# aanna0701/face-recognition-pytorch

Hardware: AMD Instinct MI355X
Metric: train imgs/sec IR-50-layout ResNet50 + ArcFace/PartialFC head, 112x112 (higher is better)
Workload: dtype bf16

## Files before the change

### face-recognition-pytorch_amd/frhip/csrc/igemm_halo.h

```cpp
#pragma once
#include <type_traits>
#include "igemm_nt.h"

#ifndef FRHIP_ABL
#define FRHIP_ABL 0
#endif

namespace frhip {

struct HaloGeom {
    int H, W, C;
    int M, Nout, Ktot;
    int sign;
    uint32_t a_bytes, b_bytes;
    const float* xf_scale;
    const float* xf_shift;
    void* xf_out;
    FastDiv d_hw, d_w;
};

template <typename T, int WM, int WN, int MT, int HBUFS>
struct HaloTile {
    static constexpr int WAVES = WM * WN, THREADS = 64 * WAVES;
    static constexpr int WROWS = MT * 16, BM = WM * WROWS, BN = WN * 64;
    static constexpr int BKE = NT_ROWB / (int)sizeof(T);
    static constexpr int MAXW = 56;
    static constexpr int HROWS = ((BM + 2 * MAXW + 2 + 7) / 8) * 8;
    static constexpr int ZROW = HROWS * NT_ROWB;
    static constexpr int HALO_BYTES = ZROW + NT_ROWB;
    static constexpr int WBUF_BYTES = BN * NT_ROWB;
    static constexpr int DUMP_OFF = HBUFS * HALO_BYTES;
    static constexpr int W_OFF = DUMP_OFF + 1024;
    static constexpr int WRING = 3;
    static constexpr int B_PIECES = (BN / 8 + WAVES - 1) / WAVES;
    static constexpr int ITER_PIECES = B_PIECES + (HBUFS == 2 ? 1 : 0);
    template <typename TS> static constexpr int stage_pitch() { return 64 * (int)sizeof(TS) + 16; }
    template <typename TS> static constexpr int lds_bytes() {
        constexpr int loop = W_OFF + WRING * WBUF_BYTES;
        constexpr int epi = WAVES * WROWS * stage_pitch<TS>();
        return loop > epi ? loop : epi;
    }
};

template <typename T, int WM, int WN, int MT, int HBUFS, bool XF = false>
struct HaloMainloop {
    static_assert(!XF || (HBUFS == 1 && std::is_same<T, bf16_t>::value), "operand transform: single-buffer bf16 tile only");
    typedef HaloTile<T, WM, WN, MT, HBUFS> Tile;
    typedef typename Mma<T>::Frag Frag;
    static constexpr int BM = Tile::BM, BN = Tile::BN, BKE = Tile::BKE;

    f32x4_t acc[4][MT];

    __device__ __forceinline__ void run(const HaloGeom& g, const void* __restrict__ a_ptr,
                                        const void* __restrict__ b_ptr, char* smem, int mtile, int ntile) {
        const int lane = lane_id(), wave = wave_id();
        const int wm = wave / WN, wn = wave % WN;
        const __amdgpu_buffer_rsrc_t ra = make_rsrc(a_ptr, g.a_bytes);
        const __amdgpu_buffer_rsrc_t rb = make_rsrc(b_ptr, g.b_bytes);
        const int m0 = mtile * BM;
        const int hrows = BM + 2 * g.W + 2;
        const int npieces = (hrows + 7) >> 3;
        const int p_lo = m0 - g.W - 1;
        const int sub = lane >> 3;
        const uint32_t chunk_bytes = (uint32_t)(((lane & 7) ^ sub) * 16);
        const int nchunks = g.C / BKE;

        const uint32_t row0_off = (uint32_t)((p_lo + sub) * g.C) * (uint32_t)sizeof(T) + chunk_bytes;
        auto halo_piece = [&](int hb, int piece, int c0) {
            const uint32_t off = row0_off + (uint32_t)(piece * 8 * g.C + c0) * (uint32_t)sizeof(T);
            glds16(ra, smem + hb * Tile::HALO_BYTES + piece * 1024, off);
        };
        auto xform_chunk = [&](int c0) {
            if constexpr (XF) {
                const int lc = (lane & 7) ^ sub;
                float sc[8], sh[8];
#pragma unroll
                for (int e = 0; e < 8; ++e) { sc[e] = g.xf_scale[c0 + 8 * lc + e]; sh[e] = g.xf_shift[c0 + 8 * lc + e]; }
                const bool emit = g.xf_out != nullptr && ntile == 0;
                for (int piece = wave; piece < npieces; piece += Tile::WAVES) {
                    const int p = p_lo + piece * 8 + sub;
                    if (p >= 0 && p < g.M) {
                        bf16x8_t* a = reinterpret_cast<bf16x8_t*>(smem + piece * 1024 + lane * 16);
                        bf16x8_t v = *a;
#pragma unroll
                        for (int e = 0; e < 8; ++e) { const float o = (float)v[e] * sc[e] + sh[e]; v[e] = (bf16_t)fmaxf(o, 0.f); }
                        *a = v;
                        if (emit && p >= m0 && p < m0 + BM)
                            *reinterpret_cast<bf16x8_t*>(reinterpret_cast<bf16_t*>(g.xf_out) + (size_t)p * g.C + c0 + 8 * lc) = v;
                    }
                }
                asm volatile("s_waitcnt lgkmcnt(0)" ::: "memory");
            }
        };
        uint32_t brow_off[Tile::B_PIECES];
#pragma unroll
        for (int j = 0; j < Tile::B_PIECES; ++j) {
            const int piece = wave * Tile::B_PIECES + j;
            const int n = ntile * BN + piece * 8 + sub;
            brow_off[j] = (piece * 8 < BN && n < g.Nout) ? (uint32_t)n * (uint32_t)g.Ktot * (uint32_t)sizeof(T) + chunk_bytes
                                                         : OOB_OFFSET;
        }
        auto weights = [&](int wit) {
            const int ch = wit / 9, tap = wit - ch * 9;
            const bool live = ch < nchunks;
            const uint32_t kb = (uint32_t)(tap * g.C + ch * BKE) * (uint32_t)sizeof(T);
            char* wb = smem + Tile::W_OFF + (wit % Tile::WRING) * Tile::WBUF_BYTES;
#pragma unroll
            for (int j = 0; j < Tile::B_PIECES; ++j) {
                const int piece = wave * Tile::B_PIECES + j;
                const bool in_tile = piece * 8 < BN;
                glds16(rb, in_tile ? wb + piece * 1024 : smem + Tile::DUMP_OFF,
                       (live && in_tile && brow_off[j] != OOB_OFFSET) ? brow_off[j] + kb : OOB_OFFSET);
            }
        };

        const int fi = lane & 15, fg = lane >> 4;
        static_assert(Tile::HALO_BYTES < 65536, "packed fragment offsets");
        uint32_t xa[9][(MT + 1) / 2];
        {
            const int HW = g.H * g.W;
            uint32_t tt[9];
#pragma unroll
            for (int tap = 0; tap < 9; ++tap) {
                const int tc = g.W + 1 + g.sign * ((tap / 3 - 1) * g.W + (tap % 3 - 1));
                tt[tap] = (uint32_t)(tc * NT_ROWB) + (uint32_t)((fg ^ ((fi + tc) & 7)) << 4);
            }
            const uint32_t zoff = (uint32_t)(Tile::ZROW + (fg << 4));
#pragma unroll
            for (int mt = 0; mt < MT; ++mt) {
                const int q = wm * Tile::WROWS + mt * 16 + fi;
                const int m = m0 + q;
                int y = 0, x = 0;
                const bool live = m < g.M;
                if (live) { const int rem = m - (int)fdiv((uint32_t)m, g.d_hw) * HW; y = (int)fdiv((uint32_t)rem, g.d_w); x = rem - y * g.W; }
                const bool up = live && y > 0, dn = live && y < g.H - 1, lf = live && x > 0, rt = live && x < g.W - 1;
                const bool vy[3] = {g.sign > 0 ? up : dn, live, g.sign > 0 ? dn : up};
                const bool vx[3] = {g.sign > 0 ? lf : rt, live, g.sign > 0 ? rt : lf};
                const uint32_t aq = (uint32_t)(q * NT_ROWB);
#pragma unroll
                for (int tap = 0; tap < 9; ++tap) {
                    const bool ok = vy[tap / 3] && vx[tap % 3];
                    const uint32_t off = ok ? aq + tt[tap] : zoff;
                    if (mt & 1) xa[tap][mt >> 1] |= off << 16;
                    else xa[tap][mt >> 1] = off;
                }
            }
        }
        const int wa = (wn * 64 + fi) * NT_ROWB + ((fg ^ (fi & 7)) << 4);

        Frag xf[2][MT], wf[2][4];
        typedef const __attribute__((address_space(3))) char* lds_cp;
        typedef const __attribute__((address_space(3))) Frag* lds_fp;
        if ((uint32_t)(uintptr_t)LDS_ADDR(smem) != 0u) __builtin_trap();
        const uint32_t wa0 = (uint32_t)wa, wa1 = (uint32_t)(wa ^ 64);
        uint32_t xcur[MT];
        auto load_frags = [&](auto set_c, auto h_c, auto hb_c, auto slot_c, auto tap_c) {
            constexpr int SET = decltype(set_c)::value, HH = decltype(h_c)::value, HB = decltype(hb_c)::value,
                          SLOT = decltype(slot_c)::value, TAP = decltype(tap_c)::value;
            (void)xf; (void)wf; (void)xcur;
#pragma unroll
            for (int t = 0; t < 4; ++t) {
                if constexpr (FRHIP_ABL & 4) asm volatile("" : "=v"(wf[SET][t]));
                else wf[SET][t] = *(lds_fp)((lds_cp)(uintptr_t)(HH ? wa1 : wa0) + (Tile::W_OFF + SLOT * Tile::WBUF_BYTES + t * 16 * NT_ROWB));
            }
#pragma unroll
            for (int mt = 0; mt < MT; ++mt) {
                if constexpr (FRHIP_ABL & 4) asm volatile("" : "=v"(xf[SET][mt]));
                else {
                    if constexpr (HH == 0) {
                        if (mt & 1) asm volatile("v_lshrrev_b32 %0, 16, %1" : "=v"(xcur[mt]) : "v"(xa[TAP][mt >> 1]));
                        else asm volatile("v_and_b32 %0, 0xffff, %1" : "=v"(xcur[mt]) : "v"(xa[TAP][mt >> 1]));
                        xf[SET][mt] = *(lds_fp)((lds_cp)(uintptr_t)xcur[mt] + HB * Tile::HALO_BYTES);
                    } else {
                        xf[SET][mt] = *(lds_fp)((lds_cp)(uintptr_t)(xcur[mt] ^ 64u) + HB * Tile::HALO_BYTES);
                    }
                }
            }
        };
        auto mfma_set = [&](auto set_c) {
            constexpr int SET = decltype(set_c)::value;
#pragma unroll
            for (int mt = 0; mt < MT; ++mt)
#pragma unroll
                for (int nt = 0; nt < 4; ++nt) {
                    if constexpr (FRHIP_ABL & 2) { Frag fa = wf[SET][nt], fb = xf[SET][mt]; asm volatile("" :: "v"(fa), "v"(fb)); }
                    else Mma<T>::run(wf[SET][nt], xf[SET][mt], acc[nt][mt]);
                }
        };
        auto mfma_set_first = [&](auto set_c) {
            constexpr int SET = decltype(set_c)::value;
#pragma unroll
            for (int mt = 0; mt < MT; ++mt)
#pragma unroll
                for (int nt = 0; nt < 4; ++nt) {
                    f32x4_t z = f32x4_t{0.f, 0.f, 0.f, 0.f};
                    if constexpr (FRHIP_ABL & 2) { Frag fa = wf[SET][nt], fb = xf[SET][mt]; asm volatile("" :: "v"(fa), "v"(fb)); }
                    else Mma<T>::run(wf[SET][nt], xf[SET][mt], z);
                    acc[nt][mt] = z;
                }
        };
        auto interleave = [&]() {
            constexpr int NREAD = (4 + MT) * (int)(sizeof(Frag) / 16), NMFMA = 4 * MT * (sizeof(T) == 2 ? 1 : (sizeof(T) == 1 ? 2 : 4));
            constexpr int PER = NMFMA / NREAD > 0 ? NMFMA / NREAD : 1;
#pragma unroll
            for (int i = 0; i < NREAD; ++i) {
                __builtin_amdgcn_sched_group_barrier(0x008, PER, 0);
                __builtin_amdgcn_sched_group_barrier(0x100, 1, 0);
            }
        };
        typedef std::integral_constant<int, 0> I0;
        typedef std::integral_constant<int, 1> I1;

        if (threadIdx.x < 8 * HBUFS) {
            const int hbz = threadIdx.x >> 3;
            *reinterpret_cast<f32x4_t*>(smem + hbz * Tile::HALO_BYTES + Tile::ZROW + (threadIdx.x & 7) * 16) = f32x4_t{0.f, 0.f, 0.f, 0.f};
        }
        for (int piece = wave; piece < npieces; piece += Tile::WAVES) halo_piece(0, piece, 0);
        weights(0);
        weights(1);
        asm volatile("s_waitcnt vmcnt(0)" ::: "memory");
        xform_chunk(0);
        __syncthreads();
        load_frags(I0{}, I0{}, I0{}, I0{}, I0{});

        auto chunk_body = [&](auto hb_c, int ch) {
            constexpr int HB = decltype(hb_c)::value;
            constexpr int HBN = HBUFS == 2 ? (HB ^ 1) : 0;
            const int c0 = ch * BKE;
            const int it0 = ch * 9;
            auto tap_body = [&](auto tap_c) {
                constexpr int TAP = decltype(tap_c)::value;
                if constexpr (!(FRHIP_ABL & 8)) {
                    weights(it0 + TAP + 2);
                    if (HBUFS == 2) {
                        const int piece = TAP * Tile::WAVES + wave;
                        if (TAP < 8 && ch + 1 < nchunks && piece < npieces) halo_piece(HBN, piece, c0 + BKE);
                        else glds16(ra, smem + Tile::DUMP_OFF, OOB_OFFSET);
                    }
                }
                load_frags(I1{}, I1{}, hb_c, std::integral_constant<int, TAP % Tile::WRING>{}, tap_c);
                if (TAP == 0 && ch == 0) mfma_set_first(I0{});
                else mfma_set(I0{});
                interleave();
                if constexpr (FRHIP_ABL & 8) asm volatile("s_waitcnt vmcnt(0)" ::: "memory");
                else if constexpr (Tile::ITER_PIECES == 1) asm volatile("s_waitcnt vmcnt(1)" ::: "memory");
                else if constexpr (Tile::ITER_PIECES == 2) asm volatile("s_waitcnt vmcnt(2)" ::: "memory");
                else if constexpr (Tile::ITER_PIECES == 3) asm volatile("s_waitcnt vmcnt(3)" ::: "memory");
                else if constexpr (Tile::ITER_PIECES == 4) asm volatile("s_waitcnt vmcnt(4)" ::: "memory");
                else asm volatile("s_waitcnt vmcnt(5)" ::: "memory");
                static_assert(Tile::ITER_PIECES <= 5, "add a vmcnt case");
                if constexpr (!(FRHIP_ABL & 1)) __builtin_amdgcn_s_barrier();
                if constexpr (TAP < 8)
                    load_frags(I0{}, I0{}, hb_c, std::integral_constant<int, (TAP + 1) % Tile::WRING>{}, std::integral_constant<int, (TAP + 1) % 9>{});
                else
                    load_frags(I0{}, I0{}, std::integral_constant<int, HBN>{}, I0{}, I0{});
                mfma_set(I1{});
                interleave();
            };
            tap_body(std::integral_constant<int, 0>{}); tap_body(std::integral_constant<int, 1>{});
            tap_body(std::integral_constant<int, 2>{}); tap_body(std::integral_constant<int, 3>{});
            tap_body(std::integral_constant<int, 4>{}); tap_body(std::integral_constant<int, 5>{});
            tap_body(std::integral_constant<int, 6>{}); tap_body(std::integral_constant<int, 7>{});
            tap_body(std::integral_constant<int, 8>{});
            if (HBUFS == 1 && ch + 1 < nchunks) {
                asm volatile("s_waitcnt lgkmcnt(0)" ::: "memory");
                __builtin_amdgcn_s_barrier();
                for (int piece = wave; piece < npieces; piece += Tile::WAVES) halo_piece(0, piece, c0 + BKE);
                asm volatile("s_waitcnt vmcnt(0)" ::: "memory");
                xform_chunk(c0 + BKE);
                __builtin_amdgcn_s_barrier();
                load_frags(I0{}, I0{}, I0{}, I0{}, I0{});
            }
        };
        static_assert(HBUFS == 1 || Tile::HROWS / 8 <= 8 * Tile::WAVES, "eight halo slices must cover the halo");
        for (int ch = 0; ch < nchunks; ch += HBUFS) {
            chunk_body(std::integral_constant<int, 0>{}, ch);
            if (HBUFS == 2 && ch + 1 < nchunks) chunk_body(std::integral_constant<int, HBUFS - 1>{}, ch + 1);
        }
        asm volatile("s_waitcnt vmcnt(0)" ::: "memory");
    }

    template <typename TS>
    __device__ __forceinline__ char* stage_out(char* smem) {
        constexpr int P = Tile::template stage_pitch<TS>();
        const int lane = lane_id();
        const int fi = lane & 15, fg = lane >> 4;
        char* mine = smem + wave_id() * Tile::WROWS * P;
        __syncthreads();
#pragma unroll
        for (int nt = 0; nt < 4; ++nt)
#pragma unroll
            for (int mt = 0; mt < MT; ++mt) {
                char* p = mine + (mt * 16 + fi) * P + (nt * 16 + 4 * fg) * (int)sizeof(TS);
                if constexpr (sizeof(TS) == 4) {
                    *reinterpret_cast<f32x4_t*>(p) = acc[nt][mt];
                } else {
                    bf16x4_t v;
#pragma unroll
                    for (int e = 0; e < 4; ++e) v[e] = (bf16_t)acc[nt][mt][e];
                    *reinterpret_cast<bf16x4_t*>(p) = v;
                }
            }
        __syncthreads();
        return mine;
    }
};

}
```

### face-recognition-pytorch_amd/frhip/csrc/igemm_halo.hip

```cpp
#include "igemm_halo.h"
#include "igemm_halo_wide.h"
#include "frhip.h"

namespace frhip {

#ifndef FRHIP_CLOCK_STAMP
#define FRHIP_CLOCK_STAMP 0
#endif
#if FRHIP_CLOCK_STAMP
__device__ unsigned long long g_clock_stamps[2 * 8192];
#endif

template <typename T, int WM, int WN, int MT, int HBUFS, bool XF = false, bool LEAN = false>
__device__ __forceinline__ void halo_body(const HaloGeom& g, const void* __restrict__ a, const void* __restrict__ b,
                                          void* __restrict__ out, const void* __restrict__ res, float* __restrict__ stats,
                                          const EpiBnRed& br, char* smem, int mtile, int ntile) {
    typedef HaloTile<T, WM, WN, MT, HBUFS> Tile;
    HaloMainloop<T, WM, WN, MT, HBUFS, XF> ml;
#if FRHIP_CLOCK_STAMP
    const unsigned long long t0 = __builtin_amdgcn_s_memtime(), r0 = __builtin_amdgcn_s_memrealtime();
#endif
    ml.run(g, a, b, smem, mtile, ntile);
#if FRHIP_CLOCK_STAMP
    if (threadIdx.x == 0) {
// ... 50 lines not shown
    const int ntile = (int)(lin % (uint32_t)ntiles), mtile = (int)(lin / (uint32_t)ntiles);
    const int m_tile0 = mtile * Tile::BM;
    HaloWideMainloop ml;
#if FRHIP_CLOCK_STAMP
    const unsigned long long t0 = __builtin_amdgcn_s_memtime(), r0 = __builtin_amdgcn_s_memrealtime();
#endif
    ml.run(g, a, b, smem, m_tile0, ntile);
#if FRHIP_CLOCK_STAMP
    if (threadIdx.x == 0) {
        const unsigned long long t1 = __builtin_amdgcn_s_memtime(), r1 = __builtin_amdgcn_s_memrealtime();
        g_clock_stamps[2 * (blockIdx.x & 8191)] = t1 - t0;
        g_clock_stamps[2 * (blockIdx.x & 8191) + 1] = r1 - r0;
    }
#endif
    const int m0 = m_tile0 + wave_id() * Tile::WROWS;
#pragma unroll
    for (int half = 0; half < 2; ++half) {
        const int n0 = ntile * Tile::BN + half * 64;
        EpiOperands<T, Tile::WROWS> eo;
        if constexpr (LEAN) {
            eo.fetch_fast(res, stats ? br.y : nullptr, g.M, g.Nout, m0, n0);
            const char* mine = ml.stage_out(smem, half);
            nt_epilogue_store_fast<T, 4, 1, Tile::WROWS, Tile::THREADS, 64>(mine, Tile::stage_pitch, smem, g.M, g.Nout, out, res != nullptr,
                                                                            stats, br, eo, mtile, ntile * 2 + half);
        } else {
            eo.fetch(res, (stats || br.gelu_bwd) ? br.y : nullptr, g.M, g.Nout, m0, n0, br.res_h, br.res_w, &br.map);
            const char* mine = ml.stage_out(smem, half);
            nt_epilogue_store<T, 4, 1, Tile::WROWS, Tile::THREADS, 64>(mine, Tile::stage_pitch, smem, g.M, g.Nout, out, res != nullptr,
                                                                       stats, br, eo, mtile, ntile * 2 + half, m0, n0);
        }
    }
}

int g_epi_lean = 1;

static int halo_wide_launch(const HaloGeom& g, const void* a, const void* b, void* out, const void* res, float* stats,
                            const EpiBnRed& br, hipStream_t stream) {
    typedef HaloWideTile Tile;
    const int mtiles = (g.M + Tile::BM - 1) / Tile::BM, ntiles = (g.Nout + Tile::BN - 1) / Tile::BN;
    const bool lean = g_epi_lean && epi_lean_ok(true, g.M, g.Nout, Tile::BM, Tile::BN, br);
    auto kern = lean ? halo_wide_kernel<true> : halo_wide_kernel<false>;
    if (set_dynamic_lds(reinterpret_cast<const void*>(kern), Tile::LDS, "igemm_halo")) return FRHIP_ELAUNCH;
    hipLaunchKernelGGL(kern, dim3(mtiles * ntiles), dim3(Tile::THREADS), Tile::LDS, stream, g, a, b, out, res, stats, br, mtiles, ntiles);
    return check_launch("igemm_halo_wide");
}

template <typename T, int WM, int WN, int MT, int HBUFS, bool XF = false>
static int halo_launch(const HaloGeom& g, const void* a, const void* b, void* out, const void* res, float* stats,
                       const EpiBnRed& br, hipStream_t stream) {
    typedef HaloTile<T, WM, WN, MT, HBUFS> Tile;
    const int mtiles = (g.M + Tile::BM - 1) / Tile::BM, ntiles = (g.Nout + Tile::BN - 1) / Tile::BN;
    const int lds = Tile::template lds_bytes<T>();
    constexpr bool HAS_LEAN = sizeof(T) == 2 && WM == 4 && WN == 1 && MT == 4 && HBUFS == 1;
    bool lean = false;
    if constexpr (HAS_LEAN) lean = g_epi_lean && epi_lean_ok(true, g.M, g.Nout, Tile::BM, Tile::BN, br);
    auto kern = halo_kernel<T, WM, WN, MT, HBUFS, XF, false>;
    if constexpr (HAS_LEAN) { if (lean) kern = halo_kernel<T, WM, WN, MT, HBUFS, XF, true>; }
    if (set_dynamic_lds(reinterpret_cast<const void*>(kern), lds, "igemm_halo")) return FRHIP_ELAUNCH;
    hipLaunchKernelGGL(kern, dim3(mtiles * ntiles), dim3(Tile::THREADS), lds, stream, g, a, b, out, res, stats, br, mtiles, ntiles);
    return check_launch("igemm_halo");
}

static int g_halo_enabled = 1;

bool halo_applicable(int dtype, int h, int w, int c, int k, int r, int s, int stride, int pad) {
    const int bke = NT_ROWB / (dtype == FRHIP_DT_BF16 ? 2 : 4);
    return g_halo_enabled && r == 3 && s == 3 && stride == 1 && pad == 1 && w <= 56 && (c % bke) == 0 && (k % 8) == 0 &&
           (dtype == FRHIP_DT_BF16 || dtype == FRHIP_DT_F32);
}

static int g_halo_wide_dirs = 2;
static int halo_config(int dtype, int c, int k);
static int halo_config_w(int dtype, int w, int c, int k, int sign) {
    if ((g_halo_wide_dirs & (sign > 0 ? 1 : 2)) && dtype == FRHIP_DT_BF16 && w <= HaloWideTile::MAXW &&
        (k % 128) == 0 && (c % 64) == 0 && c >= 128 && (g_halo_enabled & 3) == 1)
        return 3;
    return halo_config(dtype, c, k);
}
static int halo_config(int dtype, int c, int k) {
    const int es = dtype == FRHIP_DT_BF16 ? 2 : 4;
    const int nchunks = c / (NT_ROWB / es);
    const bool narrow = (k % 128) != 0;
    if (dtype == FRHIP_DT_BF16) {
        const int mode = g_halo_enabled & 3;
        const bool two_per_cu = mode == 2 || (mode != 3 && nchunks <= 8);
        if (two_per_cu || narrow) return (nchunks == 1 || two_per_cu) ? 0 : 1;
        return 2;
    }
    return narrow ? 1 : 2;
}

bool halo_lean_applies(int dtype, int n, int h, int w, int c, int k, int sign) {
    if (!g_epi_lean || dtype != FRHIP_DT_BF16) return false;
    const long long M = 1LL * n * h * w;
    const int cfg = halo_config_w(dtype, w, c, k, sign) == 3 ? 3 : halo_config(dtype, c, k);
    const int bn = cfg == 3 ? HaloWideTile::BN : 64;
    if (cfg != 3 && cfg != 0) return false;
    return M % 256 == 0 && k % bn == 0 && M * k * 2 < 0x7fffffffLL;
}

int halo_stat_rows(int, int m, int, int, int, int) { return (m + 255) / 256; }

bool halo_xf_applicable(int dtype, int h, int w, int c, int k, int r, int s, int stride, int pad) {
    return dtype == FRHIP_DT_BF16 && halo_applicable(dtype, h, w, c, k, r, s, stride, pad) && halo_config(dtype, c, k) == 0;
}

int halo_run(int dtype, const void* a, const void* b, void* out, const void* res, float* stats, const EpiBnRed& br,
             int n, int h, int w, int c, int k, int sign, hipStream_t stream, const float* xf_scale, const float* xf_shift, void* xf_out) {
    const int es = dtype == FRHIP_DT_BF16 ? 2 : 4;
    const long long ab = 1LL * n * h * w * c * es, bb = 1LL * k * 9 * c * es;
    if (ab > 0x7fffffffLL || bb > 0x7fffffffLL) { set_error("igemm_halo: tensor exceeds the 2 GiB buffer window"); return FRHIP_EINVAL; }
    HaloGeom g;
    g.H = h; g.W = w; g.C = c; g.M = n * h * w; g.Nout = k; g.Ktot = 9 * c; g.sign = sign;
    g.a_bytes = (uint32_t)ab; g.b_bytes = (uint32_t)bb;
    g.xf_scale = xf_scale; g.xf_shift = xf_shift; g.xf_out = xf_out;
    g.d_hw = make_fastdiv((uint32_t)(h * w)); g.d_w = make_fastdiv((uint32_t)w);
    const int cfg = halo_config(dtype, c, k);
    if (xf_scale) {
        if (dtype != FRHIP_DT_BF16 || cfg != 0) { set_error("igemm_halo: operand transform not available for this shape"); return FRHIP_EINVAL; }
        return halo_launch<bf16_t, 4, 1, 4, 1, true>(g, a, b, out, res, stats, br, stream);
    }
    if (halo_config_w(dtype, w, c, k, sign) == 3) return halo_wide_launch(g, a, b, out, res, stats, br, stream);
    if (dtype == FRHIP_DT_BF16 && cfg == 0) return halo_launch<bf16_t, 4, 1, 4, 1>(g, a, b, out, res, stats, br, stream);
    return by_dtype(dtype, "igemm_halo", [&](auto t) {
        typedef decltype(t) T;
        return cfg == 1 ? halo_launch<T, 8, 1, 2, 2>(g, a, b, out, res, stats, br, stream)
                        : halo_launch<T, 4, 2, 4, 2>(g, a, b, out, res, stats, br, stream);
    });
}

}

#if FRHIP_CLOCK_STAMP
extern "C" int frhip_dbg_clock_read(unsigned long long* host, int pairs) {
    if (pairs > 8192) pairs = 8192;
    return hipMemcpyFromSymbol(host, HIP_SYMBOL(frhip::g_clock_stamps), sizeof(unsigned long long) * 2 * pairs) == hipSuccess ? 0 : -1;
}
#endif

extern "C" int frhip_set_epi_lean(int enabled) {
    const int old = frhip::g_epi_lean;
    if (enabled >= 0) frhip::g_epi_lean = enabled != 0;
    return old;
}

extern "C" int frhip_set_halo_wide_dirs(int dirs) {
    const int old = frhip::g_halo_wide_dirs;
    if (dirs >= 0) frhip::g_halo_wide_dirs = dirs & 3;
    return old;
}

extern "C" int frhip_set_conv_halo(int enabled) {
    const int old = frhip::g_halo_enabled;
    frhip::g_halo_enabled = enabled & 3;
    return old;
}
```

### face-recognition-pytorch_amd/frhip/csrc/igemm_nt.h

```cpp
#pragma once
#include "common.h"

namespace frhip {

struct NtGeom {
    int H, W, C;
    int Ho, Wo;
    int R, S, stride, pad;
    int mode;
    int M, Nout, Ktot;
    int ksteps, ksteps_per_split;
    uint32_t a_bytes, b_bytes;
    int par_a, par_b, hc, wc, par_r0, par_s0;
};

struct OutMap {
    int hc, wc, ho, wo, a, b;
    __device__ __forceinline__ long long row(int m) const {
        if (wc == 0) return m;
        const int per = hc * wc;
        const int img = m / per, rem = m - img * per;
        const int i = rem / wc, j = rem - i * wc;
        return ((long long)img * ho + 2 * i + a) * wo + 2 * j + b;
    }
};

constexpr int NT_ROWB = 128;

struct EpiBnRed {
    const void* y;
    const float* mean;
    const float* invstd;
    const float* mscale;
    const float* mshift;
    int res_h, res_w;
    OutMap map;
    const float* bias;
    void* act;
    int gelu_bwd;
    const float* aff_scale;
    const float* aff_shift;
    int aff_relu;
    const float* rowkeep;
    int rows_per;
    float keep_scale;
};

template <typename T, int WM, int WN, int MT = 4>
struct NtTile {
    static constexpr int WAVES = WM * WN, THREADS = 64 * WAVES;
    static constexpr int WROWS = MT * 16;
    static constexpr int BM = WM * WROWS, BN = WN * 64;
    static constexpr int BKE = NT_ROWB / (int)sizeof(T);
    static constexpr int STAGE_BYTES = (BM + BN) * NT_ROWB;
    static constexpr int A_PIECES = BM / 8 / WAVES, B_PIECES = BN / 8 / WAVES;
// ... 536 lines not shown
                                                  const EpiBnRed& br, const EpiOperands<T, WROWS>& ops, int mtile,
                                                  int ntile, int m0, int n0) {
    constexpr int EPV = 16 / (int)sizeof(T);
    constexpr int LPR = 64 / EPV;
    constexpr int RPI = 64 / LPR;
    const int lane = lane_id(), wave = wave_id();
    const int chunk = lane % LPR, rsub = lane / LPR;
    const int n = n0 + chunk * EPV;
    float s1[EPV], s2[EPV];
#pragma unroll
    for (int e = 0; e < EPV; ++e) { s1[e] = 0.f; s2[e] = 0.f; }
    T* o = reinterpret_cast<T*>(out);
    if (stats && br.y && !br.gelu_bwd) {
        float mu[EPV], is[EPV], ms[EPV], mb[EPV];
#pragma unroll
        for (int e = 0; e < EPV; ++e) {
            const bool ok = n + e < Nout;
            mu[e] = ok ? br.mean[n + e] : 0.f; is[e] = ok ? br.invstd[n + e] : 0.f;
            ms[e] = (ok && br.mscale) ? br.mscale[n + e] : 0.f; mb[e] = (ok && br.mscale) ? br.mshift[n + e] : 1.f;
        }
#pragma unroll
        for (int it = 0; it < WROWS / RPI; ++it) {
            const int row = it * RPI + rsub;
            const int m = m0 + row;
            Vec16<T> v = *reinterpret_cast<const Vec16<T>*>(mine + row * P + chunk * 16);
            if (m < M && n < Nout) {
                if (has_res) {
                    const Vec16<T> rr = ops.res_row(it);
#pragma unroll
                    for (int e = 0; e < EPV; ++e) v.set(e, v.get(e) + rr.get(e));
                }
                epi_store_row(o + (size_t)br.map.row(m) * Nout + n, v);
                const Vec16<T> yr = ops.y_row(it);
                const float kf = br.rowkeep ? (br.rowkeep[m / br.rows_per] != 0.f ? br.keep_scale : 0.f) : 1.f;
#pragma unroll
                for (int e = 0; e < EPV; ++e) {
                    const float yy = yr.get(e);
                    const float d = (yy * ms[e] + mb[e] > 0.f) ? v.get(e) * kf : 0.f;
                    s1[e] += d; s2[e] += d * (yy - mu[e]) * is[e];
                }
            }
        }
    } else {
        float bb[EPV];
#pragma unroll
        for (int e = 0; e < EPV; ++e) bb[e] = (br.bias && n + e < Nout) ? br.bias[n + e] : 0.f;
        T* ao = reinterpret_cast<T*>(br.act);
#pragma unroll
        for (int it = 0; it < WROWS / RPI; ++it) {
            const int row = it * RPI + rsub;
            const int m = m0 + row;
            Vec16<T> v = *reinterpret_cast<const Vec16<T>*>(mine + row * P + chunk * 16);
            if (m < M && n < Nout) {
                if (has_res) {
                    const Vec16<T> rr = ops.res_row(it);
#pragma unroll
                    for (int e = 0; e < EPV; ++e) v.set(e, v.get(e) + rr.get(e));
                }
                if (br.bias) {
#pragma unroll
                    for (int e = 0; e < EPV; ++e) v.set(e, v.get(e) + bb[e]);
                }
                if (br.gelu_bwd) {
                    const Vec16<T> hv = ops.y_row(it);
#pragma unroll
                    for (int e = 0; e < EPV; ++e) {
                        v.set(e, v.get(e) * gelu_slope<T>(hv.get(e)));
// ... 48 lines not shown
```

### face-recognition-pytorch_amd/frhip/csrc/igemm_nt.hip

```cpp
#include "igemm_nt.h"
#include "frhip.h"

namespace frhip {

bool halo_applicable(int dtype, int h, int w, int c, int k, int r, int s, int stride, int pad);
int halo_stat_rows(int dtype, int m, int w, int c, int k, int sign);
bool halo_xf_applicable(int dtype, int h, int w, int c, int k, int r, int s, int stride, int pad);
bool halo_lean_applies(int dtype, int n, int h, int w, int c, int k, int sign);
int halo_run(int dtype, const void* a, const void* b, void* out, const void* res, float* stats, const EpiBnRed& br,
             int n, int h, int w, int c, int k, int sign, hipStream_t stream, const float* xf_scale = nullptr,
             const float* xf_shift = nullptr, void* xf_out = nullptr);

enum { EPI_STORE = 0, EPI_ATOMIC = 1, EPI_SLAB = 2, EPI_LEAN = 3 };
extern int g_epi_lean;

template <typename T, int WM, int WN, int MT, int EPI>
__device__ __forceinline__ void nt_tile(const NtGeom& g, const void* __restrict__ a, const void* __restrict__ b, void* __restrict__ out,
                                        const void* __restrict__ res, float* __restrict__ stats, const EpiBnRed& br, int ntiles,
                                        uint32_t t, uint32_t total, char* smem) {
    typedef NtTile<T, WM, WN, MT> Tile;
    constexpr int WROWS = Tile::WROWS, THREADS = Tile::THREADS;
    const uint32_t lin = xcd_remap(t, total);
    const int ntile = (int)(lin % (uint32_t)ntiles), mtile = (int)(lin / (uint32_t)ntiles);
    const int ks_begin = blockIdx.y * g.ksteps_per_split;
    const int ks_end = min(g.ksteps, ks_begin + g.ksteps_per_split);

    NtMainloop<T, WM, WN, MT> ml;
    ml.run(g, a, b, smem, mtile, ntile, ks_begin, ks_end);

    const int lane = lane_id(), wave = wave_id();
    const int wm = wave / WN, wn = wave % WN;
    const int m0 = mtile * Tile::BM + wm * WROWS, n0 = ntile * Tile::BN + wn * 64;

    if constexpr (EPI == EPI_LEAN) {
        if (stats && br.y && !br.gelu_bwd) {
            constexpr int P = Tile::template stage_pitch<T>();
            float accs[2][4] = {{0.f, 0.f, 0.f, 0.f}, {0.f, 0.f, 0.f, 0.f}};
#pragma unroll
            for (int half = 0; half < 2; ++half) {
                EpiOperands<T, 64> eo;
                eo.fetch_fast(res, br.y, g.M, g.Nout, m0 + 64 * half, n0);
// ... 109 lines not shown
        return FRHIP_EINVAL;
    }
    const long long a_bytes = 1LL * n * h * w * c * esize(dtype), b_bytes = 1LL * k * r * s * c * esize(dtype);
    if (a_bytes > 0x7fffffffLL || b_bytes > 0x7fffffffLL || 1LL * n * ho * wo > 0x7fffffffLL) {
        set_error("%s: tensor exceeds the 2 GiB buffer-addressing window", who);
        return FRHIP_EINVAL;
    }
    g.H = h; g.W = w; g.C = c; g.Ho = ho; g.Wo = wo; g.R = r; g.S = s; g.stride = stride; g.pad = pad; g.mode = mode;
    g.M = n * ho * wo; g.Nout = k; g.Ktot = r * s * c;
    g.ksteps = r * s * (c / bke); g.ksteps_per_split = g.ksteps;
    g.a_bytes = (uint32_t)a_bytes; g.b_bytes = (uint32_t)b_bytes;
    g.par_a = -1; g.par_b = -1; g.hc = 0; g.wc = 0; g.par_r0 = 0; g.par_s0 = 0;
    return FRHIP_OK;
}

static bool dgrad_by_parity(const NtGeom& g) { return g.mode == 1 && g.stride == 2 && g.R == 3 && g.S == 3 && g.pad == 1; }

static int nt_block_rows(int dtype, const NtGeom& g) {
    static const int bm_of[5] = {128, 128, 256, 256, 256};
    return bm_of[nt_pick_tile(dtype, g)];
}

static int parity_class(const NtGeom& g, int dtype, int a, int b, NtGeom& gc, OutMap& map) {
    gc = g;
    gc.par_a = a; gc.par_b = b;
    gc.hc = (g.Ho - a + 1) / 2; gc.wc = (g.Wo - b + 1) / 2;
    gc.par_r0 = (a + g.pad) & 1; gc.par_s0 = (b + g.pad) & 1;
    const int nr = (g.R - gc.par_r0 + 1) / 2, ns = (g.S - gc.par_s0 + 1) / 2;
    const int n_img = g.M / (g.Ho * g.Wo);
    gc.M = n_img * gc.hc * gc.wc;
    gc.ksteps = nr * ns * (g.C / (NT_ROWB / (dtype == FRHIP_DT_BF16 ? 2 : 4)));
    gc.ksteps_per_split = gc.ksteps;
    map.hc = gc.hc; map.wc = gc.wc; map.ho = g.Ho; map.wo = g.Wo; map.a = a; map.b = b;
    return gc.M;
}

}

using namespace frhip;

extern "C" int frhip_nt_block_m(int nout) {
    return ((nout % 128) == 0 || nout > 256) ? 128 : 256;
}
extern "C" int frhip_conv_stat_rows(int dtype, int m, int k, int h, int w, int c, int r, int s, int stride, int pad) {
    if (halo_applicable(dtype, h, w, c, k, r, s, stride, pad)) return halo_stat_rows(dtype, m, w, c, k, +1);
    NtGeom g; g.M = m; g.Nout = k;
    static const int bm_of[5] = {128, 128, 256, 256, 256};
    const int bm = bm_of[nt_pick_tile(dtype, g)];
    return (m + bm - 1) / bm;
}
extern "C" int frhip_set_nt_tile(int tile) { const int old = g_nt_tile; g_nt_tile = tile; return old; }

extern "C" int frhip_conv_fwd(int dtype, const void* x, const void* w, void* y, float* stats_partial,
                              int n, int h, int wd, int c, int k, int r, int s, int stride, int pad,
                              hipStream_t stream) {
    if (const int rc = by_dtype(dtype, "frhip_conv_fwd", [](auto) { return FRHIP_OK; })) return rc;
    NtGeom g;
    const int ho = (h + 2 * pad - r) / stride + 1, wo = (wd + 2 * pad - s) / stride + 1;
    int rc = fill_geom(g, dtype, n, h, wd, c, ho, wo, k, r, s, stride, pad, 0, "frhip_conv_fwd");
    if (rc) return rc;
    if (halo_applicable(dtype, h, wd, c, k, r, s, stride, pad))
        return halo_run(dtype, x, w, y, nullptr, stats_partial, NO_BNRED, n, h, wd, c, k, +1, stream);
    return nt_dispatch(dtype, g, x, w, y, nullptr, stats_partial, NO_BNRED, 1, false, stream);
}

extern "C" int frhip_conv_fwd_affine(int dtype, const void* x, const void* w, void* y, const float* scale, const float* shift, int relu,
// ... 9 lines not shown
        EpiBnRed br = NO_BNRED;
        br.aff_scale = scale; br.aff_shift = shift; br.aff_relu = relu;
        return halo_run(dtype, x, w, y, residual, nullptr, br, n, h, wd, c, k, +1, stream);
    }
    rc = frhip_conv_fwd(dtype, x, w, y, nullptr, n, h, wd, c, k, r, s, stride, pad, stream);
    if (rc) return rc;
    return frhip_bn_apply(dtype, y, scale, shift, residual, nullptr, nullptr, relu, y, n * ho * wo, k, stream);
}

extern "C" int frhip_conv_bnrelu_fusable(int dtype, int h, int wd, int c, int k, int r, int s, int stride, int pad) {
    return halo_xf_applicable(dtype, h, wd, c, k, r, s, stride, pad) ? 1 : 0;
}

extern "C" int frhip_conv_fwd_bnrelu(int dtype, const void* x, const float* in_scale, const float* in_shift, const void* w, void* y,
                                     float* stats_partial, void* act_out, int n, int h, int wd, int c, int k, int r, int s, int stride,
                                     int pad, hipStream_t stream) {
    if (const int rc = by_dtype(dtype, "frhip_conv_fwd_bnrelu", [](auto) { return FRHIP_OK; })) return rc;
    if (!in_scale || !in_shift || !halo_xf_applicable(dtype, h, wd, c, k, r, s, stride, pad)) {
        set_error("frhip_conv_fwd_bnrelu: not fusable for this shape (ask frhip_conv_bnrelu_fusable first)");
        return FRHIP_EINVAL;
    }
    return halo_run(dtype, x, w, y, nullptr, stats_partial, NO_BNRED, n, h, wd, c, k, +1, stream, in_scale, in_shift, act_out);
}

static int dgrad_run(int dtype, const void* dy, const void* wt, void* dx, const void* residual, float* stats,
                     const EpiBnRed& br, int n, int h, int wd, int c, int k, int r, int s, int stride, int pad,
                     hipStream_t stream, const char* who) {
    NtGeom g;
    const int ho = (h + 2 * pad - r) / stride + 1, wo = (wd + 2 * pad - s) / stride + 1;
    int rc = fill_geom(g, dtype, n, ho, wo, k, h, wd, c, r, s, stride, pad, 1, who);
    if (rc) return rc;
    if (halo_applicable(dtype, h, wd, k, c, r, s, stride, pad))
        return halo_run(dtype, dy, wt, dx, residual, stats, br, n, h, wd, k, c, -1, stream);
    if (dgrad_by_parity(g)) {
        float* st = stats;
        for (int cls = 0; cls < 4; ++cls) {
            NtGeom gc; EpiBnRed bc = br;
            if (parity_class(g, dtype, cls >> 1, cls & 1, gc, bc.map) == 0) continue;
            rc = nt_dispatch(dtype, gc, dy, wt, dx, residual, st, bc, 1, false, stream);
            if (rc) return rc;
            if (st) st += (size_t)((gc.M + nt_block_rows(dtype, gc) - 1) / nt_block_rows(dtype, gc)) * 2 * gc.Nout;
        }
        return FRHIP_OK;
    }
    return nt_dispatch(dtype, g, dy, wt, dx, residual, stats, br, 1, false, stream);
}

extern "C" int frhip_conv_dgrad(int dtype, const void* dy, const void* wt, void* dx, const void* residual,
                                int n, int h, int wd, int c, int k, int r, int s, int stride, int pad,
                                hipStream_t stream) {
    if (const int rc = by_dtype(dtype, "frhip_conv_dgrad", [](auto) { return FRHIP_OK; })) return rc;
    return dgrad_run(dtype, dy, wt, dx, residual, nullptr, NO_BNRED, n, h, wd, c, k, r, s, stride, pad, stream, "frhip_conv_dgrad");
}

extern "C" int frhip_dgrad_stat_rows(int dtype, int n, int h, int wd, int c, int k, int r, int s, int stride, int pad) {
    const int m = n * h * wd;
    if (halo_applicable(dtype, h, wd, k, c, r, s, stride, pad)) return halo_stat_rows(dtype, m, wd, k, c, -1);
    NtGeom g; g.M = m; g.Nout = c;
    g.mode = 1; g.stride = stride; g.R = r; g.S = s; g.pad = pad; g.Ho = h; g.Wo = wd; g.C = k;
    if (dgrad_by_parity(g)) {
        int rows = 0;
        for (int cls = 0; cls < 4; ++cls) {
            NtGeom gc; OutMap map;
            const int mc = parity_class(g, dtype, cls >> 1, cls & 1, gc, map);
            rows += (mc + nt_block_rows(dtype, gc) - 1) / nt_block_rows(dtype, gc);
        }
        return rows;
    }
    const int bm = nt_block_rows(dtype, g);
    return (m + bm - 1) / bm;
}

extern "C" int frhip_conv_dgrad_fused(int dtype, const void* dy, const void* wt, void* dx, const void* residual,
                                      int residual_stride, const void* y_bn, const float* mean, const float* invstd,
                                      const float* mask_scale, const float* mask_shift, float* stats_partial, int n, int h,
                                      int wd, int c, int k, int r, int s, int stride, int pad, hipStream_t stream) {
    if (const int rc = by_dtype(dtype, "frhip_conv_dgrad_fused", [](auto) { return FRHIP_OK; })) return rc;
    if (residual_stride != 1 && residual_stride != 2) { set_error("frhip_conv_dgrad_fused: residual_stride must be 1 or 2"); return FRHIP_EINVAL; }
    if (y_bn && (!mean || !invstd || !stats_partial || (mask_scale && !mask_shift))) {
        set_error("frhip_conv_dgrad_fused: y_bn needs mean, invstd and stats_partial");
        return FRHIP_EINVAL;
    }
    EpiBnRed br = {y_bn, mean, invstd, mask_scale, mask_shift, 0, 0, {0, 0, 0, 0, 0, 0}, nullptr, nullptr, 0};
    if (residual && residual_stride == 2) { br.res_h = h; br.res_w = wd; }
    return dgrad_run(dtype, dy, wt, dx, residual, y_bn ? stats_partial : nullptr, br, n, h, wd, c, k, r, s, stride, pad, stream,
                     "frhip_conv_dgrad_fused");
}

extern "C" int frhip_conv_dgrad_fused_rs(int dtype, const void* dy, const void* wt, void* dx, const void* residual,
                                         int residual_stride, const void* y_bn, const float* mean, const float* invstd,
// ... 97 lines not shown
```

### include/frhip.h

```cpp
#ifndef FRHIP_H
#define FRHIP_H
#include <stddef.h>
#include <stdint.h>

#ifdef __cplusplus
extern "C" {
#endif

#ifndef FRHIP_STREAM_T
#define FRHIP_STREAM_T
#ifdef __HIP_PLATFORM_AMD__
#include <hip/hip_runtime_api.h>
typedef hipStream_t frhip_stream_t;
#else
typedef void* frhip_stream_t;
#endif
#endif

#define FRHIP_OK 0
#define FRHIP_EINVAL (-1)
#define FRHIP_ELAUNCH (-2)
#define FRHIP_DT_BF16 0
#define FRHIP_DT_F32 1

const char* frhip_last_error(void);
int frhip_abi_version(void);
int frhip_spin(long long ticks, frhip_stream_t stream);

int frhip_nt_block_m(int k);
int frhip_conv_stat_rows(int dtype, int m, int k, int h, int w, int c, int r, int s, int stride, int pad);
int frhip_set_wgrad_taps9(int enabled);
int frhip_set_wgrad_mask_table(int enabled);
int frhip_wgrad_mask_table_period(int h, int w);
int frhip_set_conv_halo(int enabled);
int frhip_set_halo_wide_dirs(int dirs);
int frhip_set_epi_lean(int enabled);
int frhip_set_ew_batch(int enabled);
int frhip_set_nt_tile(int tile);
int frhip_conv_fwd_affine(int dtype, const void* x, const void* w, void* y, const float* scale, const float* shift, int relu,
                          const void* residual, int n, int h, int wd, int c, int k, int r, int s, int stride, int pad,
                          frhip_stream_t stream);
int frhip_conv_fwd(int dtype, const void* x, const void* w, void* y, float* stats_partial,
                   int n, int h, int wd, int c, int k, int r, int s, int stride, int pad, frhip_stream_t stream);
int frhip_conv_dgrad(int dtype, const void* dy, const void* wt, void* dx, const void* residual,
                     int n, int h, int wd, int c, int k, int r, int s, int stride, int pad, frhip_stream_t stream);
int frhip_dgrad_stat_rows(int dtype, int n, int h, int wd, int c, int k, int r, int s, int stride, int pad);
int frhip_conv_dgrad_bnred(int dtype, const void* dy, const void* wt, void* dx, const void* residual,
                           const void* y_bn, const float* mean, const float* invstd, const float* mask_scale,
                           const float* mask_shift, float* stats_partial, int n, int h, int wd, int c, int k,
                           int r, int s, int stride, int pad, frhip_stream_t stream);
int frhip_conv_dgrad_fused(int dtype, const void* dy, const void* wt, void* dx, const void* residual, int residual_stride,
                           const void* y_bn, const float* mean, const float* invstd, const float* mask_scale,
                           const float* mask_shift, float* stats_partial, int n, int h, int wd, int c, int k,
                           int r, int s, int stride, int pad, frhip_stream_t stream);
int frhip_conv_dgrad_fused_rs(int dtype, const void* dy, const void* wt, void* dx, const void* residual, int residual_stride,
                              const void* y_bn, const float* mean, const float* invstd, const float* mask_scale,
                              const float* mask_shift, const float* rowscale, int rows_per, float keep_scale,
                              float* stats_partial, int n, int h, int wd, int c, int k, int r, int s, int stride, int pad,
                              frhip_stream_t stream);
int frhip_conv_wgrad(int dtype, const void* dy, const void* x, float* dw, int n, int h, int w, int c,
                     int k, int r, int s, int stride, int pad, int splits, float* workspace, size_t workspace_bytes,
                     frhip_stream_t stream);
int frhip_conv_wgrad_chain_ok(int dtype, int n, int h, int w, int c, int k, int r, int s, int stride, int pad);
int frhip_conv_wgrad_chain(int dtype, const void* dy, const void* x, int n, int h, int w, int c, int k, float* slabs,
                           size_t slab_bytes, float* prev_dw, const float* prev_slabs, int prev_k, int prev_c, int prev_splits,
                           int* splits_out, frhip_stream_t stream);
int frhip_conv_wgrad_chain_finish(float* dw, float* slabs, int k, int c, int splits, frhip_stream_t stream);
int frhip_wgrad_plan(int dtype, int n, int h, int w, int c, int kc, int ldp, int r, int s, int stride, int pad, int splits,
// ... 287 lines not shown
```

Measured before the change: 23360.

## Add halo-tiled stride-2 3x3 data-gradient kernel computing all four parity classes

Adds a dedicated halo kernel for the stride-2 3x3 conv data-gradient. Each tile loads a single dy halo and accumulates all four output parity classes in separate accumulator sets, then stores each class through the existing epilogue. This replaces four separate parity-class launches, each of which re-read dy and weights. It also swaps integer divides in the output-row mapping for fast divisors. In exchange, the kernel holds four times the accumulators, which adds register pressure, and the row-keep indexing in the epilogue changes to use the mapped row.

```diff
diff --git a/face-recognition-pytorch_amd/frhip/csrc/igemm_halo.h b/face-recognition-pytorch_amd/frhip/csrc/igemm_halo.h
--- a/face-recognition-pytorch_amd/frhip/csrc/igemm_halo.h
+++ b/face-recognition-pytorch_amd/frhip/csrc/igemm_halo.h
@@ -19,13 +19,13 @@
     FastDiv d_hw, d_w;
 };
 
-template <typename T, int WM, int WN, int MT, int HBUFS>
+template <typename T, int WM, int WN, int MT, int HBUFS, bool S2 = false>
 struct HaloTile {
     static constexpr int WAVES = WM * WN, THREADS = 64 * WAVES;
     static constexpr int WROWS = MT * 16, BM = WM * WROWS, BN = WN * 64;
     static constexpr int BKE = NT_ROWB / (int)sizeof(T);
     static constexpr int MAXW = 56;
-    static constexpr int HROWS = ((BM + 2 * MAXW + 2 + 7) / 8) * 8;
+    static constexpr int HROWS = ((BM + (S2 ? 1 : 2) * MAXW + 2 + 7) / 8) * 8;
     static constexpr int ZROW = HROWS * NT_ROWB;
     static constexpr int HALO_BYTES = ZROW + NT_ROWB;
     static constexpr int WBUF_BYTES = BN * NT_ROWB;
@@ -42,14 +42,18 @@
     }
 };
 
-template <typename T, int WM, int WN, int MT, int HBUFS, bool XF = false>
+template <typename T, int WM, int WN, int MT, int HBUFS, bool XF = false, bool S2 = false>
 struct HaloMainloop {
     static_assert(!XF || (HBUFS == 1 && std::is_same<T, bf16_t>::value), "operand transform: single-buffer bf16 tile only");
-    typedef HaloTile<T, WM, WN, MT, HBUFS> Tile;
+    static_assert(!S2 || (!XF && std::is_same<T, bf16_t>::value), "stride-2 data-gradient: bf16 only, no operand transform");
+    typedef HaloTile<T, WM, WN, MT, HBUFS, S2> Tile;
     typedef typename Mma<T>::Frag Frag;
     static constexpr int BM = Tile::BM, BN = Tile::BN, BKE = Tile::BKE;
-
-    f32x4_t acc[4][MT];
+    static constexpr int NCLS = S2 ? 4 : 1;
+    static constexpr int tap_class(int tap) { return S2 ? 2 * (tap / 3 != 1) + (tap % 3 != 1) : 0; }
+    static constexpr bool tap_first(int tap) { return S2 ? (tap == 0 || tap == 1 || tap == 3 || tap == 4) : tap == 0; }
+
+    f32x4_t acc[4 * NCLS][MT];
 
     __device__ __forceinline__ void run(const HaloGeom& g, const void* __restrict__ a_ptr,
                                         const void* __restrict__ b_ptr, char* smem, int mtile, int ntile) {
@@ -58,9 +62,9 @@
         const __amdgpu_buffer_rsrc_t ra = make_rsrc(a_ptr, g.a_bytes);
         const __amdgpu_buffer_rsrc_t rb = make_rsrc(b_ptr, g.b_bytes);
         const int m0 = mtile * BM;
-        const int hrows = BM + 2 * g.W + 2;
+        const int hrows = BM + (S2 ? 1 : 2) * g.W + 2;
         const int npieces = (hrows + 7) >> 3;
-        const int p_lo = m0 - g.W - 1;
+        const int p_lo = S2 ? m0 : m0 - g.W - 1;
         const int sub = lane >> 3;
         const uint32_t chunk_bytes = (uint32_t)(((lane & 7) ^ sub) * 16);
         const int nchunks = g.C / BKE;
@@ -122,7 +126,8 @@
             uint32_t tt[9];
 #pragma unroll
             for (int tap = 0; tap < 9; ++tap) {
-                const int tc = g.W + 1 + g.sign * ((tap / 3 - 1) * g.W + (tap % 3 - 1));
+                const int tc = S2 ? (tap / 3 == 0 ? g.W : 0) + (tap % 3 == 0 ? 1 : 0)
+                                  : g.W + 1 + g.sign * ((tap / 3 - 1) * g.W + (tap % 3 - 1));
                 tt[tap] = (uint32_t)(tc * NT_ROWB) + (uint32_t)((fg ^ ((fi + tc) & 7)) << 4);
             }
             const uint32_t zoff = (uint32_t)(Tile::ZROW + (fg << 4));
@@ -139,7 +144,7 @@
                 const uint32_t aq = (uint32_t)(q * NT_ROWB);
 #pragma unroll
                 for (int tap = 0; tap < 9; ++tap) {
-                    const bool ok = vy[tap / 3] && vx[tap % 3];
+                    const bool ok = S2 ? live && (tap / 3 != 0 || dn) && (tap % 3 != 0 || rt) : vy[tap / 3] && vx[tap % 3];
                     const uint32_t off = ok ? aq + tt[tap] : zoff;
                     if (mt & 1) xa[tap][mt >> 1] |= off << 16;
                     else xa[tap][mt >> 1] = off;
@@ -177,18 +182,18 @@
                 }
             }
         };
-        auto mfma_set = [&](auto set_c) {
-            constexpr int SET = decltype(set_c)::value;
+        auto mfma_set = [&](auto set_c, auto cls_c) {
+            constexpr int SET = decltype(set_c)::value, A0 = 4 * decltype(cls_c)::value;
 #pragma unroll
             for (int mt = 0; mt < MT; ++mt)
 #pragma unroll
                 for (int nt = 0; nt < 4; ++nt) {
                     if constexpr (FRHIP_ABL & 2) { Frag fa = wf[SET][nt], fb = xf[SET][mt]; asm volatile("" :: "v"(fa), "v"(fb)); }
-                    else Mma<T>::run(wf[SET][nt], xf[SET][mt], acc[nt][mt]);
-                }
-        };
-        auto mfma_set_first = [&](auto set_c) {
-            constexpr int SET = decltype(set_c)::value;
+                    else Mma<T>::run(wf[SET][nt], xf[SET][mt], acc[A0 + nt][mt]);
+                }
+        };
+        auto mfma_set_first = [&](auto set_c, auto cls_c) {
+            constexpr int SET = decltype(set_c)::value, A0 = 4 * decltype(cls_c)::value;
 #pragma unroll
             for (int mt = 0; mt < MT; ++mt)
 #pragma unroll
@@ -196,7 +201,7 @@
                     f32x4_t z = f32x4_t{0.f, 0.f, 0.f, 0.f};
                     if constexpr (FRHIP_ABL & 2) { Frag fa = wf[SET][nt], fb = xf[SET][mt]; asm volatile("" :: "v"(fa), "v"(fb)); }
                     else Mma<T>::run(wf[SET][nt], xf[SET][mt], z);
-                    acc[nt][mt] = z;
+                    acc[A0 + nt][mt] = z;
                 }
         };
         auto interleave = [&]() {
@@ -230,6 +235,7 @@
             const int it0 = ch * 9;
             auto tap_body = [&](auto tap_c) {
                 constexpr int TAP = decltype(tap_c)::value;
+                typedef std::integral_constant<int, tap_class(TAP)> Cls;
                 if constexpr (!(FRHIP_ABL & 8)) {
                     weights(it0 + TAP + 2);
                     if (HBUFS == 2) {
@@ -239,8 +245,8 @@
                     }
                 }
                 load_frags(I1{}, I1{}, hb_c, std::integral_constant<int, TAP % Tile::WRING>{}, tap_c);
-                if (TAP == 0 && ch == 0) mfma_set_first(I0{});
-                else mfma_set(I0{});
+                if (tap_first(TAP) && ch == 0) mfma_set_first(I0{}, Cls{});
+                else mfma_set(I0{}, Cls{});
                 interleave();
                 if constexpr (FRHIP_ABL & 8) asm volatile("s_waitcnt vmcnt(0)" ::: "memory");
                 else if constexpr (Tile::ITER_PIECES == 1) asm volatile("s_waitcnt vmcnt(1)" ::: "memory");
@@ -254,7 +260,7 @@
                     load_frags(I0{}, I0{}, hb_c, std::integral_constant<int, (TAP + 1) % Tile::WRING>{}, std::integral_constant<int, (TAP + 1) % 9>{});
                 else
                     load_frags(I0{}, I0{}, std::integral_constant<int, HBN>{}, I0{}, I0{});
-                mfma_set(I1{});
+                mfma_set(I1{}, Cls{});
                 interleave();
             };
             tap_body(std::integral_constant<int, 0>{}); tap_body(std::integral_constant<int, 1>{});
@@ -280,8 +286,9 @@
         asm volatile("s_waitcnt vmcnt(0)" ::: "memory");
     }
 
-    template <typename TS>
+    template <typename TS, int CLS = 0>
     __device__ __forceinline__ char* stage_out(char* smem) {
+        static_assert(CLS < NCLS, "parity class");
         constexpr int P = Tile::template stage_pitch<TS>();
         const int lane = lane_id();
         const int fi = lane & 15, fg = lane >> 4;
@@ -293,11 +300,11 @@
             for (int mt = 0; mt < MT; ++mt) {
                 char* p = mine + (mt * 16 + fi) * P + (nt * 16 + 4 * fg) * (int)sizeof(TS);
                 if constexpr (sizeof(TS) == 4) {
-                    *reinterpret_cast<f32x4_t*>(p) = acc[nt][mt];
+                    *reinterpret_cast<f32x4_t*>(p) = acc[4 * CLS + nt][mt];
                 } else {
                     bf16x4_t v;
 #pragma unroll
-                    for (int e = 0; e < 4; ++e) v[e] = (bf16_t)acc[nt][mt][e];
+                    for (int e = 0; e < 4; ++e) v[e] = (bf16_t)acc[4 * CLS + nt][mt][e];
                     *reinterpret_cast<bf16x4_t*>(p) = v;
                 }
             }
diff --git a/face-recognition-pytorch_amd/frhip/csrc/igemm_halo.hip b/face-recognition-pytorch_amd/frhip/csrc/igemm_halo.hip
--- a/face-recognition-pytorch_amd/frhip/csrc/igemm_halo.hip
+++ b/face-recognition-pytorch_amd/frhip/csrc/igemm_halo.hip
@@ -106,6 +106,40 @@
     }
 }
 
+typedef HaloTile<bf16_t, 4, 1, 2, 2, true> HaloS2Tile;
+
+template <int CLS, typename ML>
+__device__ __forceinline__ void halo_s2_store_class(ML& ml, const HaloGeom& g, void* __restrict__ out, const void* __restrict__ res,
+                                                    float* __restrict__ stats, const EpiBnRed& br, char* smem, int mtiles, int mtile,
+                                                    int ntile) {
+    typedef HaloS2Tile Tile;
+    typedef bf16_t T;
+    EpiBnRed bc = br;
+    bc.map.a = CLS >> 1; bc.map.b = CLS & 1;
+    const int m0 = mtile * Tile::BM + wave_id() * Tile::WROWS, n0 = ntile * Tile::BN;
+    EpiOperands<T, Tile::WROWS> eo;
+    eo.fetch(res, stats ? br.y : nullptr, g.M, g.Nout, m0, n0, br.res_h, br.res_w, &bc.map);
+    const char* mine = ml.template stage_out<T, CLS>(smem);
+    __builtin_amdgcn_s_waitcnt(0x0F70);
+    nt_epilogue_store<T, 4, 1, Tile::WROWS, Tile::THREADS, Tile::BN>(mine, Tile::template stage_pitch<T>(), smem, g.M, g.Nout, out, res != nullptr,
+                                                                     stats ? stats + (size_t)CLS * mtiles * 2 * g.Nout : nullptr, bc, eo,
+                                                                     mtile, ntile, m0, n0);
+}
+
+__global__ __launch_bounds__(256, 2) void halo_s2_kernel(HaloGeom g, const void* __restrict__ a, const void* __restrict__ b,
+                                                         void* __restrict__ out, const void* __restrict__ res,
+                                                         float* __restrict__ stats, EpiBnRed br, int mtiles, int ntiles) {
+    extern __shared__ __attribute__((aligned(16))) char smem[];
+    const uint32_t lin = xcd_remap(blockIdx.x, gridDim.x);
+    const int ntile = (int)(lin % (uint32_t)ntiles), mtile = (int)(lin / (uint32_t)ntiles);
+    HaloMainloop<bf16_t, 4, 1, 2, 2, false, true> ml;
+    ml.run(g, a, b, smem, mtile, ntile);
+    halo_s2_store_class<0>(ml, g, out, res, stats, br, smem, mtiles, mtile, ntile);
+    halo_s2_store_class<1>(ml, g, out, res, stats, br, smem, mtiles, mtile, ntile);
+    halo_s2_store_class<2>(ml, g, out, res, stats, br, smem, mtiles, mtile, ntile);
+    halo_s2_store_class<3>(ml, g, out, res, stats, br, smem, mtiles, mtile, ntile);
+}
+
 int g_epi_lean = 1;
 
 static int halo_wide_launch(const HaloGeom& g, const void* a, const void* b, void* out, const void* res, float* stats,
@@ -164,6 +198,36 @@
     return narrow ? 1 : 2;
 }
 
+static int g_dgrad_s2 = 1;
+
+bool halo_s2_applicable(int dtype, int h, int w, int c, int k, int r, int s, int stride, int pad) {
+    return g_dgrad_s2 && g_halo_enabled && dtype == FRHIP_DT_BF16 && r == 3 && s == 3 && stride == 2 && pad == 1 && (h % 2) == 0 &&
+           (w % 2) == 0 && w / 2 <= HaloS2Tile::MAXW && (k % 64) == 0 && (c % 64) == 0;
+}
+
+int halo_s2_stat_rows(int n, int h, int w) { return 4 * ((n * (h / 2) * (w / 2) + HaloS2Tile::BM - 1) / HaloS2Tile::BM); }
+
+int halo_s2_run(const void* dy, const void* b, void* dx, const void* res, float* stats, const EpiBnRed& br, int n, int h, int w, int c,
+                int k, hipStream_t stream) {
+    typedef HaloS2Tile Tile;
+    const int hd = h / 2, wd = w / 2;
+    const long long ab = 1LL * n * hd * wd * k * 2, bb = 1LL * c * 9 * k * 2;
+    if (ab > 0x7fffffffLL || bb > 0x7fffffffLL) { set_error("igemm_halo: tensor exceeds the 2 GiB buffer window"); return FRHIP_EINVAL; }
+    HaloGeom g;
+    g.H = hd; g.W = wd; g.C = k; g.M = n * hd * wd; g.Nout = c; g.Ktot = 9 * k; g.sign = -1;
+    g.a_bytes = (uint32_t)ab; g.b_bytes = (uint32_t)bb;
+    g.xf_scale = nullptr; g.xf_shift = nullptr; g.xf_out = nullptr;
+    g.d_hw = make_fastdiv((uint32_t)(hd * wd)); g.d_w = make_fastdiv((uint32_t)wd);
+    const int mtiles = (g.M + Tile::BM - 1) / Tile::BM, ntiles = g.Nout / Tile::BN;
+    const int lds = Tile::lds_bytes<bf16_t>();
+    EpiBnRed bm = br;
+    bm.map.hc = hd; bm.map.wc = wd; bm.map.ho = h; bm.map.wo = w; bm.map.a = 0; bm.map.b = 0;
+    bm.map.set_divisors();
+    if (set_dynamic_lds(reinterpret_cast<const void*>(halo_s2_kernel), lds, "igemm_halo_s2")) return FRHIP_ELAUNCH;
+    hipLaunchKernelGGL(halo_s2_kernel, dim3(mtiles * ntiles), dim3(Tile::THREADS), lds, stream, g, dy, b, dx, res, stats, bm, mtiles, ntiles);
+    return check_launch("igemm_halo_s2");
+}
+
 bool halo_lean_applies(int dtype, int n, int h, int w, int c, int k, int sign) {
     if (!g_epi_lean || dtype != FRHIP_DT_BF16) return false;
     const long long M = 1LL * n * h * w;
@@ -224,6 +288,12 @@
     return old;
 }
 
+extern "C" int frhip_set_dgrad_s2(int mode) {
+    const int old = frhip::g_dgrad_s2;
+    if (mode >= 0) frhip::g_dgrad_s2 = mode != 0;
+    return old;
+}
+
 extern "C" int frhip_set_conv_halo(int enabled) {
     const int old = frhip::g_halo_enabled;
     frhip::g_halo_enabled = enabled & 3;
diff --git a/face-recognition-pytorch_amd/frhip/csrc/igemm_nt.h b/face-recognition-pytorch_amd/frhip/csrc/igemm_nt.h
--- a/face-recognition-pytorch_amd/frhip/csrc/igemm_nt.h
+++ b/face-recognition-pytorch_amd/frhip/csrc/igemm_nt.h
@@ -16,11 +16,13 @@
 
 struct OutMap {
     int hc, wc, ho, wo, a, b;
+    FastDiv d_per, d_wc;
+    void set_divisors() { d_per = make_fastdiv((uint32_t)(hc * wc)); d_wc = make_fastdiv((uint32_t)wc); }
     __device__ __forceinline__ long long row(int m) const {
         if (wc == 0) return m;
         const int per = hc * wc;
-        const int img = m / per, rem = m - img * per;
-        const int i = rem / wc, j = rem - i * wc;
+        const int img = (int)fdiv((uint32_t)m, d_per), rem = m - img * per;
+        const int i = (int)fdiv((uint32_t)rem, d_wc), j = rem - i * wc;
         return ((long long)img * ho + 2 * i + a) * wo + 2 * j + b;
     }
 };
@@ -623,7 +625,7 @@
                 }
                 epi_store_row(o + (size_t)br.map.row(m) * Nout + n, v);
                 const Vec16<T> yr = ops.y_row(it);
-                const float kf = br.rowkeep ? (br.rowkeep[m / br.rows_per] != 0.f ? br.keep_scale : 0.f) : 1.f;
+                const float kf = br.rowkeep ? (br.rowkeep[(int)br.map.row(m) / br.rows_per] != 0.f ? br.keep_scale : 0.f) : 1.f;
 #pragma unroll
                 for (int e = 0; e < EPV; ++e) {
                     const float yy = yr.get(e);
diff --git a/face-recognition-pytorch_amd/frhip/csrc/igemm_nt.hip b/face-recognition-pytorch_amd/frhip/csrc/igemm_nt.hip
--- a/face-recognition-pytorch_amd/frhip/csrc/igemm_nt.hip
+++ b/face-recognition-pytorch_amd/frhip/csrc/igemm_nt.hip
@@ -7,6 +7,10 @@
 int halo_stat_rows(int dtype, int m, int w, int c, int k, int sign);
 bool halo_xf_applicable(int dtype, int h, int w, int c, int k, int r, int s, int stride, int pad);
 bool halo_lean_applies(int dtype, int n, int h, int w, int c, int k, int sign);
+bool halo_s2_applicable(int dtype, int h, int w, int c, int k, int r, int s, int stride, int pad);
+int halo_s2_stat_rows(int n, int h, int w);
+int halo_s2_run(const void* dy, const void* b, void* dx, const void* res, float* stats, const EpiBnRed& br, int n, int h, int w, int c,
+                int k, hipStream_t stream);
 int halo_run(int dtype, const void* a, const void* b, void* out, const void* res, float* stats, const EpiBnRed& br,
              int n, int h, int w, int c, int k, int sign, hipStream_t stream, const float* xf_scale = nullptr,
              const float* xf_shift = nullptr, void* xf_out = nullptr);
@@ -182,6 +186,7 @@
     gc.ksteps = nr * ns * (g.C / (NT_ROWB / (dtype == FRHIP_DT_BF16 ? 2 : 4)));
     gc.ksteps_per_split = gc.ksteps;
     map.hc = gc.hc; map.wc = gc.wc; map.ho = g.Ho; map.wo = g.Wo; map.a = a; map.b = b;
+    if (gc.M > 0) map.set_divisors();
     return gc.M;
 }
 
@@ -257,6 +262,8 @@
     if (rc) return rc;
     if (halo_applicable(dtype, h, wd, k, c, r, s, stride, pad))
         return halo_run(dtype, dy, wt, dx, residual, stats, br, n, h, wd, k, c, -1, stream);
+    if (halo_s2_applicable(dtype, h, wd, c, k, r, s, stride, pad))
+        return halo_s2_run(dy, wt, dx, residual, stats, br, n, h, wd, c, k, stream);
     if (dgrad_by_parity(g)) {
         float* st = stats;
         for (int cls = 0; cls < 4; ++cls) {
@@ -281,6 +288,7 @@
 extern "C" int frhip_dgrad_stat_rows(int dtype, int n, int h, int wd, int c, int k, int r, int s, int stride, int pad) {
     const int m = n * h * wd;
     if (halo_applicable(dtype, h, wd, k, c, r, s, stride, pad)) return halo_stat_rows(dtype, m, wd, k, c, -1);
+    if (halo_s2_applicable(dtype, h, wd, c, k, r, s, stride, pad)) return halo_s2_stat_rows(n, h, wd);
     NtGeom g; g.M = m; g.Nout = c;
     g.mode = 1; g.stride = stride; g.R = r; g.S = s; g.pad = pad; g.Ho = h; g.Wo = wd; g.C = k;
     if (dgrad_by_parity(g)) {
diff --git a/include/frhip.h b/include/frhip.h
--- a/include/frhip.h
+++ b/include/frhip.h
@@ -34,6 +34,7 @@
 int frhip_wgrad_mask_table_period(int h, int w);
 int frhip_set_conv_halo(int enabled);
 int frhip_set_halo_wide_dirs(int dirs);
+int frhip_set_dgrad_s2(int mode);
 int frhip_set_epi_lean(int enabled);
 int frhip_set_ew_batch(int enabled);
 int frhip_set_nt_tile(int tile);
```

New measurement: 23320 (median of 2 runs). Within noise of the previous version (-0.2%).
